# kevslinger/DTQN

Measured on AMD Instinct MI355X. Metric: env-steps/sec + TD-updates/sec, DiscreteCarFlag-v0 ctx=50 b=32, 1/2/4/8 GPU, higher is better.
Workload: dtype f32; 1 GPU; DiscreteCarFlag-v0 shapes (BASELINE config 1): ctx=50, d_model=64, 8 heads, 2 layers, obs 3 f32, 3 actions, batch 32 per GPU, history 50, device replay 2500 x 200 steps; global_batch=32, parallelism=dp1, sampler=device

## Files before the change

### dtqn_amd/csrc/dtqn_backward.hip

```cpp
#include "dtqn_device.hpp"
#include "dtqn_bwd_device.hpp"
#include "dtqn_gru.hpp"
#include "dtqn_wgrad_direct.hpp"
#include "dtqn_forward_body.hpp"

#ifndef DTQN_SPLIT_ATTN_MFMA
#define DTQN_SPLIT_ATTN_MFMA 1
#endif
#ifndef DTQN_BWD_DOX
#define DTQN_BWD_DOX 1
#endif
#ifndef DTQN_BWD_DOX_EARLY_FLAG
#define DTQN_BWD_DOX_EARLY_FLAG 1
#endif
#ifndef DTQN_BWD_FOLD_GUARD
#define DTQN_BWD_FOLD_GUARD 0
#endif
#if DTQN_BWD_FOLD_GUARD
#define DTQN_BWD_GUARD(w, q) Own::valid_fast(w, q)
#else
#define DTQN_BWD_GUARD(w, q) Own::valid(w, q)
#endif

namespace dtqn {

struct BwdArgs {
    DtqnNet net;
    const float* theta;
    const float* act;
    float* grd;
    float* small;
    const float* q3;
    float* stats_partial;
    const float* obs;
    const uint8_t* actions;
    const float* rewards;
    const uint8_t* dones;
    long long obs_ep_stride, act_ep_stride, rew_ep_stride;
    const int32_t* ep_idx;
    const int32_t* start;
    int batch, history;
    float gamma;
    long long* prof;
    float* xch;
    int32_t* xflags;
    uint32_t drop_thresh, drop_seed;
    float drop_scale;
    const int32_t* step_counter;
    FuseArgs fuse;
};

template <bool AHEAD> struct AheadArgs {};
template <> struct AheadArgs<true> { FwdArgs f; };

template <int D, int MT, int HD, int NW, bool GRU, int RS, bool DROP, bool FUSE = false, bool AHEAD = false, bool PAD = false>
__global__ __launch_bounds__(NW * 64) void dtqn_backward_kernel(BwdArgs a, AheadArgs<AHEAD> ahead) {
    static_assert(RS == 1 || RS == 2 || RS == 4, "one, two or four row slices");
    static_assert(!PAD || (RS == 4 && MT == 1 && !GRU && !DROP && !FUSE && D == 64), "width padding rides with the four-slice residual-gate chain");
    if constexpr (AHEAD) {
        static_assert(RS == 4 && MT == 1 && !GRU && !DROP && !FUSE && D <= 64, "the target pass ahead rides with the four-slice residual-gate chain");
        if ((int)blockIdx.x >= a.batch * RS) {
            forward_body_wl<D, 1, HD, NW, 4, false, PAD>(ahead.f);
            return;
        }
    }
    constexpr int NT = NW * 64;
    constexpr int LP = MT * 16;
    constexpr int LPF = LP * RS;
    constexpr int LDX = D + 4;
    constexpr int GW = D >= 64 ? 64 : D;
    constexpr int NG = D / GW;
    constexpr int NC = D >= 128 ? D / 2 : 2 * D;
    constexpr bool OST = D <= 64;
    constexpr int W5C = ((OST ? 6 : 5) * GW > NC ? (OST ? 6 : 5) * GW : NC);
    constexpr int LD5 = W5C + 4;
    constexpr int MGX = pick_mg(D / 16, MT, NW);
    using Own = Owned<D, MT, MGX, NW>;
    const DtqnNet& net = a.net;
    const Thr t = make_thr();
    const Thr& t_outer = t;
    if constexpr (FUSE) {
        if ((int)blockIdx.x >= a.batch * RS) {
            const DirectCtx ctx{a.act, a.grd, a.small, a.fuse.grad, a.batch, RS, a.fuse.n_small};
            fuse_role<NW>(net, a.fuse, ctx, (int)blockIdx.x - a.batch * RS, reinterpret_cast<float*>(dtqn_smem), t);
            return;
        }
    }
    int b, pos;
    slice_block_map((int)blockIdx.x, a.batch, RS, b, pos);
    const int slice = RS - 1 - pos;
    const int R0 = slice * LP;
    const int Lfull = net.ctx_len, A = net.num_actions, AP = net.ap, H = net.num_heads, adim = net.action_dim;
    const int L = Lfull - R0 < LP ? Lfull - R0 : LP;
    const bool ident = RS > 1 ? false : net.identity != 0;
    const int dreal = PAD ? net.d_real : D;
    constexpr bool gru = GRU;
    const float* __restrict__ theta = a.theta;
    const float* rec = a.act + (size_t)b * net.act_stride;
    float* grec = a.grd + (size_t)b * net.grd_stride;
    float* srec = a.small + ((size_t)b * RS + slice) * net.sp_stride;
    auto rf = [&](const float* base, int off, int w) -> const float* { return base + off + (size_t)R0 * w; };
    auto gf = [&](float* base, int off, int w) -> float* { return base + off + (size_t)R0 * w; };
    auto mf = [&](const float* base, int off, int ctiles) -> const float* { return base + off + (size_t)(R0 / 16) * ctiles * 8; };
    const DtqnRsrc grs = DTQN_XCH_RSRC(grec, (size_t)net.grd_stride * 4);
    constexpr bool WT = FUSE || (kOptBwdWT && !(GRU && !DROP && MT >= 2 && NW == 8));
    auto g_store4 = [&](float* p, float4 v) {
        if constexpr (WT) dtqn_xch_store4(grs, (int)(p - grec) * 4, v);
        else st4(p, v);
    };
    auto g_tile_store = [&](const float* s_, int ld_, float* g_, int rows, int cols, int gld = 0) {
        if constexpr (WT) {
            const int c4 = cols >> 2;
            if (gld == 0) gld = cols;
            const int base = (int)(g_ - grec);
            for (int idx = t_outer.tid; idx < rows * c4; idx += NT) {
                const int r = idx / c4, c = (idx - r * c4) * 4;
                dtqn_xch_store4(grs, (base + r * gld + c) * 4, ld4(s_ + r * ld_ + c));
            }
        } else {
            tile_store<NW>(s_, ld_, g_, rows, cols, t_outer, gld);
        }
    };
    auto s_store = [&](float* p, float v) {
        if constexpr (FUSE) DTQN_AGENT_STORE(p, v);
        else *p = v;
    };

    float* DX = reinterpret_cast<float*>(dtqn_smem);
    float* T2 = DX + LP * LDX;
    float* W5 = T2 + LP * LDX;
    float* dq_s = W5 + LPF * LD5;
    float* delta_s = dq_s + LP * AP;
    float* lse_s = delta_s + (GW / HD) * LPF;
    float* red = lse_s + (GW / HD) * LPF;
    constexpr int PARTS = NT / D >= 1 ? NT / D : 1;
    float* st_s = red + PARTS * 2 * D;
    float* DU = st_s + 4 * LP;

    const int ep = a.ep_idx[b], st0 = a.start[b] + R0;
    Drop dr = drop_off();
    if constexpr (DROP) dr = Drop{a.drop_thresh, a.drop_scale, a.drop_seed, (uint32_t)a.step_counter[1], (uint32_t)b};
    int ps = 0;
    DTQN_PROF(a.prof, ps++);
    static_assert(HD <= 16 || (HD == 32 && RS == 4 && MT == 1), "delta-in-epilogue: a head inside one 16-column tile, or two tiles wide on the four-slice chain");
    constexpr bool SPLITS = kOptSplitS && MT == 1 && 2 * (D / 16) == NW && 2 * (GW / 16) == NW;
    std::conditional_t<SPLITS, StageDyWSplit<D, NW, D / 16>, StageDyW<D, MT, pick_mg(D / 16, MT, NW), NW, D / 16>> g_h1;
    g_h1.prefetch(theta + net.off_head1_w, D, t);
    TileRegs<NW, LP, D> tr;
    TileRegs<NW, LP, D> trh;
    trh.load(rf(rec, net.ao_hh, D), D, t);
    if (!ident) tr.load(rf(rec, net.ao_layer0 + (net.num_layers - 1) * net.act_layer_stride + net.al_s2, D), D, t);

    static_assert(4 * LP <= NT, "one statistics value per thread");
    auto st_fetch = [&](int l) -> float {
        const float* lr = rec + net.ao_layer0 + (size_t)l * net.act_layer_stride;
        if (t.tid >= 4 * LP) return 0.f;
        return t.tid < 2 * LP ? rf(lr, net.al_st1, 2)[t.tid] : rf(lr, net.al_st2, 2)[t.tid - 2 * LP];
    };
    float st_next = st_fetch(net.num_layers - 1);

    {
        const float* q0 = a.q3 + (((size_t)0 * a.batch + b) * LPF + R0) * AP;
        const float* q1 = a.q3 + (((size_t)1 * a.batch + b) * LPF + R0) * AP;
        const float* q2 = a.q3 + (((size_t)2 * a.batch + b) * LPF + R0) * AP;
        const float inv_count = 1.0f / ((float)a.batch * (float)a.history);
        DTQN_PROF(a.prof, 24);
        for (int idx = t.tid; idx < LP * AP; idx += NT) dq_s[idx] = 0.f;
        __syncthreads();
        DTQN_PROF(a.prof, 25);
        if (t.wave == 0)
            td_loss_wave(q0, q1, q2, AP, A, Lfull - R0, LP, a.history, a.gamma, inv_count,
                         a.actions + (size_t)ep * a.act_ep_stride + st0, a.rewards + (size_t)ep * a.rew_ep_stride + st0,
                         a.dones + (size_t)ep * a.rew_ep_stride + st0, dq_s, a.stats_partial + ((size_t)b * RS + slice) * 8, t.lane);
        DTQN_PROF(a.prof, 26);
        __syncthreads();
        DTQN_PROF(a.prof, 27);
        if constexpr (WT) {
            for (int idx = t.tid; idx < LP * AP / 4; idx += NT) g_store4(gf(grec, net.go_dq, AP) + 4 * idx, ld4(dq_s + 4 * idx));
        } else {
            for (int idx = t.tid; idx < LP * AP; idx += NT) gf(grec, net.go_dq, AP)[idx] = dq_s[idx];
        }
    }

    DTQN_PROF(a.prof, ps++);
    {
        const float* __restrict__ W2 = theta + net.off_head2_w;
        constexpr int C4 = D / 4;
#pragma unroll
        for (int k4 = 0; k4 < TileRegs<NW, LP, D>::N; ++k4) {
            const int idx4 = t.tid + k4 * NT;
            if (idx4 < LP * C4) {
                const int r = idx4 / C4, c0 = (idx4 - r * C4) * 4;
                const float hv[4] = {trh.v[k4].x, trh.v[k4].y, trh.v[k4].z, trh.v[k4].w};
                float g4[4];
#pragma unroll
                for (int e = 0; e < 4; ++e) {
                    float g = 0.f;
                    if (hv[e] > 0.f)
                        for (int c = 0; c < A; ++c) g = fmaf(dq_s[r * AP + c], W2[c * D + c0 + e], g);
                    g4[e] = g;
                }
                st4(T2 + r * LDX + c0, make_float4(g4[0], g4[1], g4[2], g4[3]));
            }
        }
    }
    __syncthreads();
    g_h1.retire();
    g_tile_store(T2, LDX, gf(grec, net.go_dhh, D), LP, D);
    if constexpr (SPLITS) g_h1.run(T2, LDX, t, red, [&](int r, int c, float v) { DX[r * LDX + c] = v; });
    else g_h1.run(T2, LDX, t, [&](int r, int c, float v) { DX[r * LDX + c] = v; });
    __syncthreads();
    DTQN_PROF(a.prof, ps++);

    for (int l = net.num_layers - 1; l >= 0; --l) {
        Thr t = t_outer;
#define DTQN_RELAUNDER() do { if constexpr (D >= 128 && MT >= 4) { DTQN_ASM_KEEP(t.tid); DTQN_ASM_KEEP(t.lane); DTQN_ASM_KEEP(t.wave); DTQN_ASM_KEEP(t.i); DTQN_ASM_KEEP(t.kq); } \
        else if constexpr (D == 64 && MT >= 2 && NW <= 8 && (RS == 1 || (GRU && RS == 2))) { int tid_ = (int)threadIdx.x; DTQN_ASM_KEEP(tid_); t.tid = tid_; t.lane = tid_ & 63; t.wave = tid_ >> 6; t.i = t.lane & 15; t.kq = t.lane >> 4; } } while (0)
        DTQN_RELAUNDER();
        const float* __restrict__ th = layer_theta(net, theta, l);
        const float* lrec = rec + net.ao_layer0 + (size_t)l * net.act_layer_stride;
        float* lgrd = grec + net.go_layer0 + (size_t)l * net.grd_layer_stride;
        float* lsm = srec + net.so_ln + l * 4 * D;
        const float* __restrict__ W1 = th + net.lo_f1_w;
        const float* __restrict__ W2 = th + net.lo_f2_w;
        StageDyW<D, MT, pick_mg(NC / 16, MT, NW), NW, NC / 16> g_dh;
        g_dh.prefetch(W2, 4 * D, t);
        if (t.tid < 4 * LP) st_s[t.tid] = st_next;
        if (l > 0) st_next = st_fetch(l - 1);

        if (!ident) {
            if (l == net.num_layers - 1) DTQN_PROF(a.prof, 28);
            tr.to_lds(T2, LDX, t);
            if (l == net.num_layers - 1) DTQN_PROF(a.prof, 29);
            __syncthreads();
            if (l == net.num_layers - 1) DTQN_PROF(a.prof, 30);
            layernorm_backward<D, NW, FUSE, PAD>(DX, T2, DX, false, LDX, LP, st_s + 2 * LP, th + net.lo_ln2_w, lsm + 2 * D, red, t, false, dreal);
            if (l == net.num_layers - 1) DTQN_PROF(a.prof, 31);
            __syncthreads();
        }
        DTQN_PROF(a.prof, ps++);
        tr.load(rf(lrec, net.al_s1, D), D, t);
        if (gru) {
            gru_gate_backward<D, MT, NW>(DX, T2, LDX, W5, LD5, theta + net.off_gate_mlp, net, lrec + net.al_gate2, lgrd + net.gl_gate2, t, LPF, R0);
            __syncthreads();
        }
        {
            const float* m2 = mf(lrec, net.al_m2, D / 16);
            for (int idx = t.tid; idx < LP * D; idx += NT) {
                const int r = idx / D, c = idx - r * D;
                const float dy = gru ? T2[r * LDX + c] : DX[r * LDX + c];
                T2[r * LDX + c] = mask_bit(m2, D / 16, r, c) ? drop_apply(dr, DROP_FFN, l, (uint32_t)((R0 + r) * D + c), dy) : 0.f;
            }
        }
        __syncthreads();
        DTQN_RELAUNDER();
        {
            f32x4 xacc[Own::PER_WAVE][MGX];
#pragma unroll
            for (int q = 0; q < Own::PER_WAVE; ++q)
#pragma unroll
                for (int m = 0; m < MGX; ++m) xacc[q][m] = zero4();
            float w1f[2][NC / 4];
            constexpr bool SPLITK = kOptSplitK && Own::ITEMS * 2 == NW && Own::PER_WAVE == 1 && MGX == 1 && NC % 32 == 0;
            constexpr bool HALFW = kOptHalfW && !SPLITK && NC % 32 == 0;
            const int sk_it = t.wave % Own::ITEMS, sk_kh = t.wave / Own::ITEMS;
            const unsigned long long* mh = reinterpret_cast<const unsigned long long*>(mf(lrec, net.al_mh, 4 * D / 16));
            constexpr int MGH = pick_mg(NC / 16, MT, NW);
#pragma clang loop unroll_count(D >= 128 ? 1 : 4)
            for (int c0 = 0; c0 < 4 * D; c0 += NC) {
                g_dh.retire();
                if (c0 == 0) g_tile_store(T2, LDX, gf(lgrd, net.gl_df, D), LP, D);
                unsigned long long mw[MGH][4];
                g_dh.run(T2, LDX, t,
                         [&](int kt, int mg) {
#pragma unroll
                             for (int m = 0; m < MGH; ++m)
#pragma unroll
                                 for (int r = 0; r < 4; ++r)
                                     mw[m][r] = mh[((mg * MGH + m) * (4 * D / 16) + (c0 >> 4) + kt) * 4 + r];
                         },
                         [&](int r, int c, float v) {
                             const unsigned long long w = mw[(r >> 4) % MGH][r & 3];
                             W5[r * LD5 + c] = ((w >> t.lane) & 1ull) ? v : 0.f;
                         });
                if constexpr (SPLITK) {
                    float (&wh)[NC / 8] = *reinterpret_cast<float (*)[NC / 8]>(&w1f[0][0]);
                    frag_dyw_fetch<NC / 2>(wh, W1 + (size_t)(c0 + sk_kh * (NC / 2)) * D + sk_it * 16 + t.i, D, t);
                } else if constexpr (HALFW) {
                    float (&wh)[NC / 8] = *reinterpret_cast<float (*)[NC / 8]>(&w1f[0][0]);
                    if (DTQN_BWD_GUARD(t.wave, 0)) frag_dyw_fetch<NC / 2>(wh, W1 + (size_t)c0 * D + Own::nt(t.wave, 0) * 16 + t.i, D, t);
                } else if (DTQN_BWD_GUARD(t.wave, 0))
                    frag_dyw_fetch<NC>(w1f[0], W1 + (size_t)c0 * D + Own::nt(t.wave, 0) * 16 + t.i, D, t);
                if constexpr (FUSE) {
                    if (c0 == 0 && l + 1 < net.num_layers) DTQN_WAIT_VMEM();
                }
                __syncthreads();
                if constexpr (FUSE) {
                    if (c0 == 0 && l + 1 < net.num_layers) fuse_arrive(a.fuse.counters, net.num_layers - 2 - l, t);
                }
                if (SPLITK || DTQN_BWD_GUARD(t.wave, 0)) {
#pragma unroll
                    for (int q = 0; q < (SPLITK || HALFW ? NC / 8 : NC / 4); ++q) DTQN_ASM_KEEP(w1f[0][q]);
                }
                g_tile_store(W5, LD5, gf(lgrd, net.gl_dhp, 4 * D) + c0, LP, NC, 4 * D);
                if constexpr (SPLITK) {
                    const float (&wh)[NC / 8] = *reinterpret_cast<const float (*)[NC / 8]>(&w1f[0][0]);
                    frag_dyw_mma<NC / 2, 1>(W5 + sk_kh * (NC / 2), LD5, wh, t, xacc[0]);
                } else if constexpr (HALFW) {
                    float (&wa)[NC / 8] = *reinterpret_cast<float (*)[NC / 8]>(&w1f[0][0]);
                    float (&wb)[NC / 8] = *reinterpret_cast<float (*)[NC / 8]>(&w1f[1][0]);
#pragma unroll
                    for (int q = 0; q < Own::PER_WAVE; ++q) {
                        const float* wcol = W1 + (size_t)c0 * D + Own::nt(t.wave, q) * 16 + t.i;
                        const float* rows = W5 + Own::mg(t.wave, q) * MGX * 16 * LD5;
                        if (DTQN_BWD_GUARD(t.wave, q)) {
                            frag_dyw_fetch<NC / 2>(wb, wcol + (size_t)(NC / 2) * D, D, t);
                            frag_dyw_mma<NC / 2, MGX>(rows, LD5, wa, t, xacc[q]);
                        }
                        if (q + 1 < Own::PER_WAVE && DTQN_BWD_GUARD(t.wave, q + 1))
                            frag_dyw_fetch<NC / 2>(wa, W1 + (size_t)c0 * D + Own::nt(t.wave, q + 1) * 16 + t.i, D, t);
                        if (DTQN_BWD_GUARD(t.wave, q)) frag_dyw_mma<NC / 2, MGX>(rows + NC / 2, LD5, wb, t, xacc[q]);
                    }
                } else {
#pragma unroll
                    for (int q = 0; q < Own::PER_WAVE; ++q) {
                        if (q + 1 < Own::PER_WAVE && DTQN_BWD_GUARD(t.wave, q + 1))
                            frag_dyw_fetch<NC>(w1f[(q + 1) & 1], W1 + (size_t)c0 * D + Own::nt(t.wave, q + 1) * 16 + t.i, D, t);
                        if (DTQN_BWD_GUARD(t.wave, q))
                            frag_dyw_mma<NC, MGX>(W5 + Own::mg(t.wave, q) * MGX * 16 * LD5, LD5, w1f[q & 1], t, xacc[q]);
                    }
                }
                if (c0 + NC < 4 * D) g_dh.prefetch(W2 + c0 + NC, 4 * D, t);
                __syncthreads();
            }
            if constexpr (SPLITK) {
                if (t.wave >= Own::ITEMS) {
#pragma unroll
                    for (int r4 = 0; r4 < 4; ++r4) W5[((t.wave - Own::ITEMS) * 4 + r4) * 64 + t.lane] = xacc[0][0][r4];
                }
                __syncthreads();
                if (t.wave < Own::ITEMS) {
#pragma unroll
                    for (int r4 = 0; r4 < 4; ++r4) xacc[0][0][r4] += W5[(t.wave * 4 + r4) * 64 + t.lane];
                }
            }
            float* dst = ident ? DU : DX;
#pragma unroll
            for (int q = 0; q < Own::PER_WAVE; ++q) {
                if (DTQN_BWD_GUARD(t.wave, q)) {
                    const int c = Own::nt(t.wave, q) * 16 + t.i;
#pragma unroll
                    for (int m = 0; m < MGX; ++m)
#pragma unroll
                        for (int r4 = 0; r4 < 4; ++r4) {
                            const int r = (Own::mg(t.wave, q) * MGX + m) * 16 + t.kq * 4 + r4;
                            if (ident) dst[r * LDX + c] = xacc[q][m][r4];
                            else dst[r * LDX + c] += xacc[q][m][r4];
                        }
                }
            }
        }
        tr.to_lds(T2, LDX, t);
        constexpr bool DOX = RS > 1 && DTQN_BWD_DOX && DTQN_SPLIT_ATTN_MFMA;
        TileRegs<NW, LP, GW> tq, to, tk[RS], tv[RS], tqu[DOX ? RS : 1];
        constexpr int NLSE = (GW / HD) * LPF, LSE_N = (NLSE + NT - 1) / NT;
        float lse_r[LSE_N];
        auto load_group = [&](int g) {
            if constexpr (kOptLse) {
#pragma unroll
                for (int k = 0; k < LSE_N; ++k) {
                    const int idx = t.tid + k * NT;
                    lse_r[k] = lrec[net.al_lse + g * NLSE + (idx < NLSE ? idx : 0)];
                }
            }
            const float* qkv0 = lrec + net.al_qkv + g * GW;
            tq.load(qkv0 + (size_t)R0 * 3 * D, 3 * D, t);
            if constexpr (DOX) {
#pragma unroll
                for (int j = 1; j < RS; ++j)
                    if (j > slice) tqu[j].load(qkv0 + (size_t)j * LP * 3 * D, 3 * D, t);
            }
#pragma unroll
            for (int j = 0; j < RS; ++j)
                if (j <= slice) {
                    tk[j].load(qkv0 + (size_t)j * LP * 3 * D + D, 3 * D, t);
                    tv[j].load(qkv0 + (size_t)j * LP * 3 * D + 2 * D, 3 * D, t);
                }
            if (OST) to.load(rf(lrec, net.al_o, D) + g * GW, D, t);
        };
        load_group(0);
        const float* __restrict__ Wo = th + net.lo_out_w;
        const float* __restrict__ Win = th + net.lo_in_w;
        std::conditional_t<SPLITS, StageDyWSplit<D, NW, GW / 16>, StageDyW<D, MT, pick_mg(GW / 16, MT, NW), NW, GW / 16>> g_do;
// ... 169 lines not shown
                        const DtqnRsrc rs = DTQN_XCH_RSRC(xg + (size_t)pair_id(slice, 0) * LP * 2 * GW, R0 * 2 * GW * 4);
                        constexpr int C4 = 2 * GW / 4;
                        for (int idx = t.tid; idx < R0 * C4; idx += NT) {
                            const int r = idx / C4, c = (idx - r * C4) * 4;
                            dtqn_xch_store4(rs, idx * 16, ld4(W5 + r * LD5 + GW + c));
                        }
                        DTQN_WAIT_VMEM();
                        __syncthreads();
                        if (t.tid < slice) DTQN_AGENT_STORE(fg + pair_id(slice, t.tid), (int32_t)1);
                    }
                    for (int sndr = slice + 1; sndr < RS; ++sndr)
                        xch_recv<NW, true>(W5r + GW, LD5, xg + (size_t)pair_id(sndr, slice) * LP * 2 * GW, LP, 2 * GW,
                                           fg + pair_id(sndr, slice), t);
                }
                }
                DTQN_PROF(a.prof, ps++);
                if constexpr (SPLITW) {
#pragma unroll
                    for (int q = 0; q < WPC / 4; ++q) DTQN_ASM_KEEP(wpc[0][q]);
                } else if (DTQN_BWD_GUARD(t.wave, 0)) {
#pragma unroll
                    for (int q = 0; q < GW / 4; ++q) DTQN_ASM_KEEP(winf[0][q]);
                }
                if (g == 0 && DOX) g_tile_store(T2, LDX, gf(lgrd, net.gl_da, D), LP, D);
                for (int idx = t.tid; idx < LP * 3 * (GW / 4); idx += NT) {
                    const int r = idx / (3 * (GW / 4)), rem = idx - r * (3 * (GW / 4));
                    const int which = rem / (GW / 4), c = (rem - which * (GW / 4)) * 4;
                    const float* sp = W5r + r * LD5 + (which == 0 ? 4 * GW : which * GW) + c;
                    g_store4(gf(lgrd, net.gl_dqkv, 3 * D) + (size_t)r * 3 * D + which * D + g * GW + c, ld4(sp));
                }
                if constexpr (SPLITW) {
#pragma unroll
                    for (int j = 0; j < 3; ++j) {
                        if (j + 1 < 3) piece_fetch(wpc[(j + 1) & 1], g, j + 1);
                        const int u = sw_kh * 3 + j, part = u >> 1, off = (u & 1) * WPC;
                        frag_dyw_mma<WPC, 1>(W5r + (part == 0 ? 4 * GW : part * GW) + off, LD5, wpc[j & 1], t, xacc[0]);
                    }
                } else
#pragma unroll
                for (int q = 0; q < Own::PER_WAVE; ++q) {
#pragma unroll
                    for (int part = 0; part < 3; ++part) {
                        const int step = q * 3 + part;
                        const int nq = part < 2 ? q : q + 1, np = part < 2 ? part + 1 : 0;
                        if (nq < Own::PER_WAVE && DTQN_BWD_GUARD(t.wave, nq))
                            frag_dyw_fetch<GW>(winf[(step + 1) & 1], Win + (size_t)(np * D + g * GW) * D + Own::nt(t.wave, nq) * 16 + t.i, D, t);
                        if (DTQN_BWD_GUARD(t.wave, q)) {
                            const float* rows = W5r + Own::mg(t.wave, q) * MGX * 16 * LD5 + (part == 0 ? 4 * GW : part * GW);
                            frag_dyw_mma<GW, MGX>(rows, LD5, winf[step & 1], t, xacc[q]);
                        }
                    }
                }
                if (g + 1 < NG) {
                    g_do.prefetch(Wo + (g + 1) * GW, D, t);
                    load_group(g + 1);
                }
                __syncthreads();
            }
            if (!ident) {
                if (l > 0) tr.load(rf(rec, net.ao_layer0 + (l - 1) * net.act_layer_stride + net.al_s2, D), D, t);
            } else {
                tr.load(l == 0 ? rf(rec, net.ao_x0, D) : rf(rec, net.ao_layer0 + (l - 1) * net.act_layer_stride + net.al_s2, D), D, t);
            }
            if constexpr (SPLITW) {
                if (t.wave >= Own::ITEMS) {
#pragma unroll
                    for (int r4 = 0; r4 < 4; ++r4) W5[((t.wave - Own::ITEMS) * 4 + r4) * 64 + t.lane] = xacc[0][0][r4];
                }
                __syncthreads();
                if (t.wave < Own::ITEMS) {
#pragma unroll
                    for (int r4 = 0; r4 < 4; ++r4) xacc[0][0][r4] += W5[(t.wave * 4 + r4) * 64 + t.lane];
                }
            }
            float* dst = ident ? DU : DX;
#pragma unroll
            for (int q = 0; q < Own::PER_WAVE; ++q) {
                if (DTQN_BWD_GUARD(t.wave, q)) {
                    const int c = Own::nt(t.wave, q) * 16 + t.i;
#pragma unroll
                    for (int m = 0; m < MGX; ++m)
#pragma unroll
                        for (int r4 = 0; r4 < 4; ++r4) {
                            const int r = (Own::mg(t.wave, q) * MGX + m) * 16 + t.kq * 4 + r4;
                            if (ident) dst[r * LDX + c] = xacc[q][m][r4];
                            else dst[r * LDX + c] += xacc[q][m][r4];
                        }
                }
            }
        }
        __syncthreads();
        DTQN_PROF(a.prof, ps++);
        if (ident) {
            tr.to_lds(T2, LDX, t);
            __syncthreads();
            layernorm_backward<D, NW, FUSE, PAD>(DU, T2, DX, true, LDX, LP, st_s, th + net.lo_ln1_w, lsm, red, t, false, dreal);
            __syncthreads();
        }
    }

    DTQN_PROF(a.prof, ps++);
    if (dr.thresh != 0u) {
        for (int idx = t.tid; idx < LP * D; idx += NT) {
            const int r = idx / D, c = idx - r * D;
            DX[r * LDX + c] = drop_apply(dr, DROP_EMB, 0, (uint32_t)((R0 + r) * D + c), DX[r * LDX + c]);
        }
        __syncthreads();
    }
    g_tile_store(DX, LDX, gf(grec, net.go_dx0, D), LP, D);
    const float* obs_rows = a.obs + (size_t)ep * a.obs_ep_stride + (size_t)st0 * net.obs_dim;
    const uint8_t* act_rows = a.actions + (size_t)ep * a.act_ep_stride + st0;
    if (net.discrete) {
        const int KE = net.ke, KEP = net.kep, e = net.embed_per_obs, V = net.vocab, O = net.obs_dim;
        const float* __restrict__ We = theta + net.off_obs_w;
        float* dein = W5;
        for (int idx = t.tid; idx < LP * KEP; idx += NT) {
            const int r = idx / KEP, k = idx - r * KEP;
            float g = 0.f;
            if (r < L && k < KE)
                for (int d = 0; d < D - adim; ++d) g = fmaf(DX[r * LDX + adim + d], We[(size_t)d * KE + k], g);
            dein[idx] = g;
        }
        __syncthreads();
        for (int idx = t.tid; idx < V * e; idx += NT) {
            const int v = idx / e, c = idx - v * e;
            float g = 0.f;
            for (int r = 0; r < L; ++r)
                for (int j = 0; j < O; ++j) {
                    int tok = (int)obs_rows[(size_t)r * O + j];
                    tok = tok < 0 ? 0 : (tok >= V ? V - 1 : tok);
                    if (tok == v) g += dein[r * KEP + j * e + c];
                }
            s_store(srec + net.so_tab + idx, g);
        }
    }
    if (adim > 0) {
        for (int idx = t.tid; idx < A * adim; idx += NT) {
            const int v = idx / adim, c = idx - v * adim;
            float g = 0.f;
            if (Lfull == 1) {
                if ((int)act_rows[0] == v) g = DX[c];
            } else {
                for (int r = R0 > 0 ? 0 : 1; r < L; ++r)
                    if ((int)act_rows[r - 1] == v) g += DX[r * LDX + c];
            }
            s_store(srec + net.so_act + idx, g);
        }
    }
    if constexpr (FUSE) {
        DTQN_WAIT_VMEM();
        __syncthreads();
        fuse_arrive(a.fuse.counters, net.num_layers, t);
    }
}

static size_t bwd_lds_bytes(const DtqnNet* net) {
    const int LP = net->lp, D = net->d_model, HD = net->head_dim;
    const int GW = D >= 64 ? 64 : D, NC = D >= 128 ? D : 2 * D;
    const int ntile = D <= 64 ? 6 : 5;
    const int W5C = ntile * GW > NC ? ntile * GW : NC;
    const int NT = waves_for(*net) * 64;
    const int PARTS = NT / D >= 1 ? NT / D : 1;
    size_t fl = 2 * (size_t)LP * (D + 4) + (size_t)LP * (W5C + 4) + (size_t)LP * net->ap + 2 * (size_t)(GW / HD) * LP +
                (size_t)PARTS * 2 * D + 4 * (size_t)LP;
    if (net->identity) fl += (size_t)LP * (D + 4);
    return fl * sizeof(float);
}

template <int D, int MT, int HD, int NW, bool GRU, int RS, bool DROP, bool FUSE = false>
static int launch_bwd3(const BwdArgs& a, hipStream_t stream) {
    const size_t lds = bwd_lds_bytes(&a.net);
    static size_t attr_lds[kMaxDevices] = {};
    raise_lds_limit(reinterpret_cast<const void*>(&dtqn_backward_kernel<D, MT, HD, NW, GRU, RS, DROP, FUSE>), lds, attr_lds);
    (void)hipGetLastError();
    const int grid = a.batch * RS + (FUSE ? a.fuse.n_role : 0);
    hipLaunchKernelGGL((dtqn_backward_kernel<D, MT, HD, NW, GRU, RS, DROP, FUSE>), dim3(grid), dim3(NW * 64), lds, stream, a, AheadArgs<false>{});
    return hipGetLastError() == hipSuccess ? DTQN_OK : DTQN_ERR_LAUNCH;
}
template <int HD, bool PAD = false>
static int launch_bwd_ahead(const BwdArgs& a, const FwdArgs& f, hipStream_t stream) {
    const size_t lb = bwd_lds_bytes(&a.net), lf = fwd_lds_bytes(&a.net, true);
    const size_t lds = lb > lf ? lb : lf;
    if (lds > 160 * 1024) return DTQN_ERR_CONFIG;
    static size_t attr_lds[kMaxDevices] = {};
    raise_lds_limit(reinterpret_cast<const void*>(&dtqn_backward_kernel<64, 1, HD, 8, false, 4, false, false, true, PAD>), lds, attr_lds);
    (void)hipGetLastError();
    AheadArgs<true> ah;
    ah.f = f;
    ah.f.block0 = a.batch * 4;
    hipLaunchKernelGGL((dtqn_backward_kernel<64, 1, HD, 8, false, 4, false, false, true, PAD>), dim3(a.batch * 4 + f.batch * 4), dim3(8 * 64), lds, stream, a, ah);
    return hipGetLastError() == hipSuccess ? DTQN_OK : DTQN_ERR_LAUNCH;
}
template <int HD, bool PAD>
static int launch_bwd_lite(const BwdArgs& a, hipStream_t stream) {
    const size_t lds = bwd_lds_bytes(&a.net);
    static size_t attr_lds[kMaxDevices] = {};
    raise_lds_limit(reinterpret_cast<const void*>(&dtqn_backward_kernel<64, 1, HD, 8, false, 4, false, false, false, PAD>), lds, attr_lds);
    (void)hipGetLastError();
    hipLaunchKernelGGL((dtqn_backward_kernel<64, 1, HD, 8, false, 4, false, false, false, PAD>), dim3(a.batch * 4), dim3(8 * 64), lds, stream, a, AheadArgs<false>{});
    return hipGetLastError() == hipSuccess ? DTQN_OK : DTQN_ERR_LAUNCH;
}
template <int D, int MT, int HD, int NW, bool GRU, int RS>
static int launch_bwd2(const BwdArgs& a, hipStream_t stream) {
    if constexpr (RS == 4 && !GRU && NW == kFuseWaves) {
        if (a.fuse.n_role > 0) {
            if (bwd_lds_bytes(&a.net) < (kFuseWaves + (size_t)(kDSmallFused / 64) * kFuseWaves * 64) * sizeof(float) ||
                bwd_lds_bytes(&a.net) < direct_lds_floats(kFuseWaves) * sizeof(float)) return DTQN_ERR_CONFIG;
            if (a.drop_thresh != 0u) return launch_bwd3<D, MT, HD, NW, GRU, RS, true, true>(a, stream);
            return launch_bwd3<D, MT, HD, NW, GRU, RS, false, true>(a, stream);
        }
    }
    if (a.fuse.n_role > 0) return DTQN_ERR_CONFIG;
    if (a.drop_thresh != 0u) return launch_bwd3<D, MT, HD, NW, GRU, RS, true>(a, stream);
    return launch_bwd3<D, MT, HD, NW, GRU, RS, false>(a, stream);
}
template <int D, int MT, int HD, int NW>
static int launch_bwd(const BwdArgs& a, hipStream_t stream) {
    if (a.net.gate == DTQN_GATE_GRU) {
        if constexpr (D <= 64) return launch_bwd2<D, MT, HD, NW, true, 1>(a, stream);
        else return DTQN_ERR_CONFIG;
    }
    return launch_bwd2<D, MT, HD, NW, false, 1>(a, stream);
}

}

using namespace dtqn;

extern "C" int dtqn_lds_bytes_backward(const DtqnNet* net) {
    if (!net) return 0;
    const size_t b = bwd_lds_bytes(net);
    return b <= 160 * 1024 ? (int)b : 0;
}

extern "C" int dtqn_td_wgrad_is_fused(const DtqnNet* net, const DtqnTd* td) {
    FuseArgs f;
    return fuse_plan(net, td, &f) ? 1 : 0;
}

static int td_backward(const DtqnNet* net, const DtqnReplay* rp, const DtqnTd* td, const DtqnTd* td_next, int draw_step_next, void* stream);

extern "C" int dtqn_td_backward(const DtqnNet* net, const DtqnReplay* rp, const DtqnTd* td, void* stream) {
    return td_backward(net, rp, td, nullptr, -1, stream);
}

extern "C" int dtqn_td_backward_ahead(const DtqnNet* net, const DtqnReplay* rp, const DtqnTd* td, const DtqnTd* td_next, int draw_step_next,
                                      void* stream) {
    if (!td_next || draw_step_next < 0) return DTQN_ERR_ARG;
    return td_backward(net, rp, td, td_next, draw_step_next, stream);
}

static int td_backward(const DtqnNet* net, const DtqnReplay* rp, const DtqnTd* td, const DtqnTd* td_next, int draw_step_next, void* stream) {
    if (!net || !rp || !td || td->batch < 1) return DTQN_ERR_ARG;
    if (td->history < 1 || td->history > net->ctx_len) return DTQN_ERR_ARG;
    if (net->tiled) return td_next ? DTQN_ERR_CONFIG : tiled_td_backward(net, rp, td, (hipStream_t)stream);
    if (bwd_lds_bytes(net) > 160 * 1024) return DTQN_ERR_CONFIG;
    BwdArgs a;
    a.net = *net;
    a.theta = td->theta_pol;
    a.act = td->act; a.grd = td->grd; a.small = td->small; a.q3 = td->q3; a.stats_partial = td->stats_partial;
    a.obs = rp->obs; a.actions = rp->actions; a.rewards = rp->rewards; a.dones = rp->dones;
    a.obs_ep_stride = (long long)(rp->max_steps + 1) * rp->obs_dim;
    a.act_ep_stride = rp->max_steps + 1;
    a.rew_ep_stride = rp->max_steps;
    a.ep_idx = td->ep_idx; a.start = td->start;
    a.batch = td->batch; a.history = td->history; a.gamma = td->gamma;
    a.prof = dtqn_debug_profile_buffer() ? static_cast<long long*>(dtqn_debug_profile_buffer()) + 64 : nullptr;
    a.xch = td->xch; a.xflags = td->xflags;
    a.drop_thresh = net->dropout > 0.f ? (uint32_t)((double)net->dropout * 4294967296.0) : 0u;
    a.drop_scale = net->dropout > 0.f ? 1.0f / (1.0f - net->dropout) : 1.0f;
    a.drop_seed = td->dropout_seed; a.step_counter = td->step_counter;
    fuse_plan(net, td, &a.fuse);
    const int D = net->d_model, MT = net->lp / 16, HD = net->head_dim, NW = waves_for(*net);
    hipStream_t s = (hipStream_t)stream;
    if (dtqn_ws_lite(net->tiled, D, HD, net->d_real)) {
        if (td->row_split != 4 || net->lp != 64 || net->identity || net->gate != DTQN_GATE_RES || !a.xch || !a.xflags || a.drop_thresh != 0u ||
            a.fuse.n_role > 0 || NW != 8) return DTQN_ERR_CONFIG;
        const bool pad = net->d_real > 0;
        if (td_next != nullptr) {
            if (!dtqn_td_fwd_slices4_ok(net) || !td_next->sample_in_kernel || td_next->batch != td->batch || !td_next->xch || !td_next->xflags ||
                !td_next->q3) return DTQN_ERR_CONFIG;
            FwdArgs f;
            td_forward_args(net, rp, td_next, 2, draw_step_next, &f);
            f.nseq = td_next->batch;
            f.prof = nullptr;
            if (HD == 8 && pad) return launch_bwd_ahead<8, true>(a, f, s);
            if (HD == 16 && pad) return launch_bwd_ahead<16, true>(a, f, s);
            if (HD == 32) return pad ? launch_bwd_ahead<32, true>(a, f, s) : launch_bwd_ahead<32, false>(a, f, s);
            return DTQN_ERR_CONFIG;
        }
        if (HD == 8 && pad) return launch_bwd_lite<8, true>(a, s);
        if (HD == 16 && pad) return launch_bwd_lite<16, true>(a, s);
        if (HD == 32) return pad ? launch_bwd_lite<32, true>(a, s) : launch_bwd_lite<32, false>(a, s);
        return DTQN_ERR_CONFIG;
    }
    if (td->row_split == 2 || td->row_split == 4) {
        if (net->lp != 64 || net->identity || !a.xch || !a.xflags) return DTQN_ERR_CONFIG;
        if (net->gate == DTQN_GATE_GRU) {
            if (td->row_split == 4) {
                if (D == 64 && HD == 8) return launch_bwd2<64, 1, 8, 8, true, 4>(a, s);
                if (D == 64 && HD == 16) return launch_bwd2<64, 1, 16, 8, true, 4>(a, s);
                return DTQN_ERR_CONFIG;
            }
            if (D == 64 && HD == 8) return launch_bwd2<64, 2, 8, 8, true, 2>(a, s);
            if (D == 64 && HD == 16) return launch_bwd2<64, 2, 16, 8, true, 2>(a, s);
            return DTQN_ERR_CONFIG;
// ... 31 lines not shown
```

### dtqn_amd/csrc/dtqn_bwd_device.hpp

```cpp
#pragma once
#include "dtqn_device.hpp"

namespace dtqn {

template <int D, int NW, bool WT = false, bool PAD = false>
__device__ __forceinline__ void layernorm_backward(const float* dy, const float* xin, float* dst, bool accumulate,
                                                   int ld, int LP, const float* __restrict__ st,
                                                   const float* __restrict__ gamma, float* __restrict__ dgb,
                                                   float* red, const Thr& t, bool dgb_accumulate = false, int d_real = D) {
    constexpr int NT = NW * 64;
    constexpr int PARTS = NT / D >= 1 ? NT / D : 1;
    {
        const int d = t.tid % D, part = t.tid / D;
        if (part < PARTS) {
            float sg = 0.f, sb = 0.f;
            for (int r = part; r < LP; r += PARTS) {
                const float mean = st[r * 2], rstd = st[r * 2 + 1];
                const float g = dy[r * ld + d];
                sg = fmaf(g, (xin[r * ld + d] - mean) * rstd, sg);
                sb += g;
            }
            red[(part * 2 + 0) * D + d] = sg;
            red[(part * 2 + 1) * D + d] = sb;
        }
// ... 230 lines not shown
    bool one_round = nblocks <= NW && (64 % HG) == 0;
    int nlive = ((q_hi > row0 ? q_hi - row0 : 0) * HG + 63) / 64;
    for (int it0 = t.tid; it0 < (one_round ? NW * 64 : LP * HG); it0 += NW * 64) {
        int item = it0;
        if (one_round) {
            const int blk = balanced_block<NW>(t.wave, nblocks, nlive, false);
            if (blk < 0) continue;
            item = blk * 64 + t.lane;
            if (item >= LP * HG) continue;
        }
        const int rl = item / HG, hl = item - rl * HG;
        const int row = row0 + rl;
        float* dqp = dq_base + (size_t)row * dq_ld + hl * HD;
        float dq[HD];
#pragma unroll
        for (int c = 0; c < HD; ++c) dq[c] = 0.f;
        if (row < n) {
            const float* qp = W5 + row * ld + hl * HD;
            const float* dop = W5 + row * ld + 3 * GW + hl * HD;
            float q[HD], dO[HD];
#pragma unroll
            for (int c = 0; c < HD; c += 4) {
                const float4 x = ld4(qp + c), g = ld4(dop + c);
                q[c] = x.x * scale; q[c + 1] = x.y * scale; q[c + 2] = x.z * scale; q[c + 3] = x.w * scale;
                dO[c] = g.x; dO[c + 1] = g.y; dO[c + 2] = g.z; dO[c + 3] = g.w;
            }
            const float delta = delta_s[hl * sl_ld + row], lse = lse_s[hl * sl_ld + row];
            const float* kbase = W5 + GW + hl * HD;
            for (int s = 0; s <= row; ++s) {
                const float* kp = kbase + s * ld;
                const float* vp = kp + GW;
                float sc = 0.f, dp = 0.f;
                float kk[HD];
#pragma unroll
                for (int c = 0; c < HD; c += 4) {
                    const float4 k = ld4(kp + c), v = ld4(vp + c);
                    kk[c] = k.x; kk[c + 1] = k.y; kk[c + 2] = k.z; kk[c + 3] = k.w;
                    sc = fmaf(q[c], k.x, sc); sc = fmaf(q[c + 1], k.y, sc); sc = fmaf(q[c + 2], k.z, sc); sc = fmaf(q[c + 3], k.w, sc);
                    dp = fmaf(dO[c], v.x, dp); dp = fmaf(dO[c + 1], v.y, dp); dp = fmaf(dO[c + 2], v.z, dp); dp = fmaf(dO[c + 3], v.w, dp);
                }
                if (dr.thresh != 0u) dp = drop_keep(dr, DROP_ATTN, layer, drop_attn_idx(head0 + hl, row, s)) ? dp * dr.scale : 0.f;
                const float ds = __expf(sc - lse) * (dp - delta);
#pragma unroll
                for (int c = 0; c < HD; ++c) dq[c] = fmaf(ds, kk[c], dq[c]);
            }
        }
#pragma unroll
        for (int c = 0; c < HD; c += 4)
            st4(dqp + c, make_float4(dq[c] * scale, dq[c + 1] * scale, dq[c + 2] * scale, dq[c + 3] * scale));
    }
    __syncthreads();
    const int KR = row0 + LP;
    nblocks = (KR * HG + 63) / 64;
    one_round = nblocks <= NW && (64 % HG) == 0;
    nlive = ((q_hi < KR ? q_hi : KR) * HG + 63) / 64;
    for (int it0 = t.tid; it0 < (one_round ? NW * 64 : KR * HG); it0 += NW * 64) {
        int item = it0;
        if (one_round) {
            const int blk = balanced_block<NW>(t.wave, nblocks, nlive, true);
            if (blk < 0) continue;
            item = blk * 64 + t.lane;
            if (item >= KR * HG) continue;
        }
        const int srow = item / HG, hl = item - srow * HG;
        float* kp = W5 + srow * ld + GW + hl * HD;
        float* vp = kp + GW;
        float dk[HD], dv[HD];
#pragma unroll
        for (int c = 0; c < HD; ++c) dk[c] = dv[c] = 0.f;
        if (srow < q_hi) {
            float k[HD], v[HD];
#pragma unroll
            for (int c = 0; c < HD; c += 4) {
                const float4 x = ld4(kp + c), y = ld4(vp + c);
                k[c] = x.x; k[c + 1] = x.y; k[c + 2] = x.z; k[c + 3] = x.w;
                v[c] = y.x; v[c + 1] = y.y; v[c + 2] = y.z; v[c + 3] = y.w;
            }
            const int q_lo = srow > row0 ? srow : row0;
            for (int row = q_hi - 1; row >= q_lo; --row) {
                const float* qp = W5 + row * ld + hl * HD;
                const float* dop = qp + 3 * GW;
                float sc = 0.f, dp = 0.f;
                float qq[HD], dd[HD];
#pragma unroll
                for (int c = 0; c < HD; c += 4) {
                    const float4 x = ld4(qp + c), g = ld4(dop + c);
                    qq[c] = x.x * scale; qq[c + 1] = x.y * scale; qq[c + 2] = x.z * scale; qq[c + 3] = x.w * scale;
                    dd[c] = g.x; dd[c + 1] = g.y; dd[c + 2] = g.z; dd[c + 3] = g.w;
                }
#pragma unroll
                for (int c = 0; c < HD; ++c) { sc = fmaf(qq[c], k[c], sc); dp = fmaf(dd[c], v[c], dp); }
                float p = __expf(sc - lse_s[hl * sl_ld + row]);
                float pv = p;
                if (dr.thresh != 0u) {
                    const bool keep = drop_keep(dr, DROP_ATTN, layer, drop_attn_idx(head0 + hl, row, srow));
                    dp = keep ? dp * dr.scale : 0.f;
                    pv = keep ? p * dr.scale : 0.f;
                }
                const float ds = p * (dp - delta_s[hl * sl_ld + row]);
#pragma unroll
                for (int c = 0; c < HD; ++c) { dk[c] = fmaf(ds, qq[c], dk[c]); dv[c] = fmaf(pv, dd[c], dv[c]); }
            }
        }
#pragma unroll
        for (int c = 0; c < HD; c += 4) {
            st4(kp + c, make_float4(dk[c], dk[c + 1], dk[c + 2], dk[c + 3]));
            st4(vp + c, make_float4(dv[c], dv[c + 1], dv[c + 2], dv[c + 3]));
        }
    }
}

template <int HD, int NW, bool MFMA = (HD >= kAttnMfmaMinHeadDim)>
__device__ __forceinline__ void attention_backward_group(float* W5, int ld, int GW, int LP, int n,
                                                         const float* delta_s, const float* lse_s, const Thr& t,
                                                         float* dq_base = nullptr, int dq_ld = 0, int row0 = 0, int sl_ld = 0,
                                                         const Drop& dr = Drop{0u, 1.0f, 0u, 0u, 0u}, int layer = 0, int head0 = 0,
                                                         float hd_eff = (float)HD) {
    if constexpr (MFMA)
        attention_backward_group_mfma<HD, NW>(W5, ld, GW, LP, n, delta_s, lse_s, t, dq_base, dq_ld, row0, sl_ld, dr, layer, head0, false, 0,
                                              AttnNoBetween(), hd_eff);
    else attention_backward_group_valu<HD, NW>(W5, ld, GW, LP, n, delta_s, lse_s, t, dq_base, dq_ld, row0, sl_ld, dr, layer, head0, hd_eff);
}

__device__ __forceinline__ void td_loss_wave(const float* q0, const float* q1, const float* q2, int AP, int A, int L, int LPB,
                                             int history, float gamma, float inv_count, const uint8_t* act, const float* rew,
                                             const uint8_t* don, float* dq, float* sp, int lane) {
    float sq = 0.f, mnq = INFINITY, mxq = -INFINITY, sy = 0.f, mny = INFINITY, mxy = -INFINITY, se = 0.f;
    for (int r = lane; r < LPB; r += 64) {
        if (r < L && r >= L - history) {
            const int at = (int)act[r];
            const float rw = rew[r];
            const float dn = don[r] ? 1.f : 0.f;
            float q = 0.f, best = q1[r * AP], qt = q2[r * AP];
            for (int c = 0; c < A; ++c) {
                const float v0 = q0[r * AP + c], v1 = q1[r * AP + c], v2 = q2[r * AP + c];
                if (c == at) q = v0;
                if (c > 0 && v1 > best) { best = v1; qt = v2; }
            }
            const float y = rw + (1.f - dn) * (qt * gamma);
            const float diff = q - y;
            dq[r * AP + at] = 2.f * diff * inv_count;
            sq += q; mnq = fminf(mnq, q); mxq = fmaxf(mxq, q);
            sy += y; mny = fminf(mny, y); mxy = fmaxf(mxy, y);
            se = fmaf(diff, diff, se);
        }
    }
    sq = wave_sum(sq); sy = wave_sum(sy); se = wave_sum(se);
    mnq = wave_min(mnq); mxq = wave_max(mxq); mny = wave_min(mny); mxy = wave_max(mxy);
    if (lane == 0) {
        sp[0] = se; sp[1] = sq; sp[2] = mxq; sp[3] = mnq; sp[4] = sy; sp[5] = mxy; sp[6] = mny; sp[7] = 0.f;
    }
}

}
```

Measured before the change: 12170 TD-updates/s.

## Split TD loss into early load issue and late finish; stage head.2 weights in LDS

The TD-loss global loads (Q values, actions, rewards, dones) are issued at kernel entry so they overlap the weight prefetches, and the loss is computed later from registers. This drops the separate dq zero-fill pass and one barrier, since each lane now writes its whole dq row. The head.2 weight matrix is staged in LDS, and the head gradient is computed as a float4 FMA with the ReLU mask applied afterwards instead of a per-element branch. Profiling timestamps are collected into a local clock array and written out at kernel end. The trade-off is extra register pressure from holding the loss operands across the prefetch phase.

```diff
diff --git a/dtqn_amd/csrc/dtqn_backward.hip b/dtqn_amd/csrc/dtqn_backward.hip
--- a/dtqn_amd/csrc/dtqn_backward.hip
+++ b/dtqn_amd/csrc/dtqn_backward.hip
@@ -140,8 +140,26 @@
     const int ep = a.ep_idx[b], st0 = a.start[b] + R0;
     Drop dr = drop_off();
     if constexpr (DROP) dr = Drop{a.drop_thresh, a.drop_scale, a.drop_seed, (uint32_t)a.step_counter[1], (uint32_t)b};
-    int ps = 0;
-    DTQN_PROF(a.prof, ps++);
+    enum { PK_ENTRY, PK_PREFETCH, PK_LOSS_LOADS, PK_LOSS_WAVE, PK_LOSS_BARRIER, PK_LOSS, PK_HEAD2, PK_HEAD, PK_DH_PREFETCH,
+           PK_STATS, PK_S2_BEFORE, PK_S2_LDS, PK_S2_BARRIER, PK_LN2_BODY, PK_LN2, PK_N };
+    long long pclk[PK_N] = {};
+    int ps = 4;
+    DTQN_PROF_CLOCK(pclk[PK_ENTRY]);
+    static_assert(LP <= 64, "one loss row per lane of one wave");
+    const float* q0 = a.q3 + (((size_t)0 * a.batch + b) * LPF + R0) * AP;
+    const float* q1 = a.q3 + (((size_t)1 * a.batch + b) * LPF + R0) * AP;
+    const float* q2 = a.q3 + (((size_t)2 * a.batch + b) * LPF + R0) * AP;
+    TdLossRow lrow = {};
+    if (t.wave == 0)
+        td_loss_issue(lrow, q0, q1, q2, AP, Lfull - R0, LP, a.history, -R0,
+                      a.actions + (size_t)ep * a.act_ep_stride + st0, a.rewards + (size_t)ep * a.rew_ep_stride + st0,
+                      a.dones + (size_t)ep * a.rew_ep_stride + st0, t.lane);
+    DTQN_SCHED_FENCE();
+    DTQN_PROF_CLOCK(pclk[PK_LOSS_LOADS]);
+    const float* __restrict__ W2h = theta + net.off_head2_w;
+    const int h2n4 = A * (D / 4);
+    static_assert(LPF * LD5 >= DTQN_MAX_ACTIONS * D, "head.2 fits the wide temp");
+    const float4 h2 = ld4(W2h + 4 * (t.tid < h2n4 ? t.tid : 0));
     static_assert(HD <= 16 || (HD == 32 && RS == 4 && MT == 1), "delta-in-epilogue: a head inside one 16-column tile, or two tiles wide on the four-slice chain");
     constexpr bool SPLITS = kOptSplitS && MT == 1 && 2 * (D / 16) == NW && 2 * (GW / 16) == NW;
     std::conditional_t<SPLITS, StageDyWSplit<D, NW, D / 16>, StageDyW<D, MT, pick_mg(D / 16, MT, NW), NW, D / 16>> g_h1;
@@ -160,21 +178,15 @@
     float st_next = st_fetch(net.num_layers - 1);
 
     {
-        const float* q0 = a.q3 + (((size_t)0 * a.batch + b) * LPF + R0) * AP;
-        const float* q1 = a.q3 + (((size_t)1 * a.batch + b) * LPF + R0) * AP;
-        const float* q2 = a.q3 + (((size_t)2 * a.batch + b) * LPF + R0) * AP;
         const float inv_count = 1.0f / ((float)a.batch * (float)a.history);
-        DTQN_PROF(a.prof, 24);
-        for (int idx = t.tid; idx < LP * AP; idx += NT) dq_s[idx] = 0.f;
+        DTQN_PROF_CLOCK(pclk[PK_PREFETCH]);
+        if (t.wave == 0)
+            td_loss_finish(lrow, q0, q1, q2, AP, A, LP, a.gamma, inv_count, dq_s, a.stats_partial + ((size_t)b * RS + slice) * 8, t.lane);
+        DTQN_PROF_CLOCK(pclk[PK_LOSS_WAVE]);
+        if (t.tid < h2n4) st4(W5 + 4 * t.tid, h2);
+        for (int idx = t.tid + NT; idx < h2n4; idx += NT) st4(W5 + 4 * idx, ld4(W2h + 4 * idx));
         __syncthreads();
-        DTQN_PROF(a.prof, 25);
-        if (t.wave == 0)
-            td_loss_wave(q0, q1, q2, AP, A, Lfull - R0, LP, a.history, a.gamma, inv_count,
-                         a.actions + (size_t)ep * a.act_ep_stride + st0, a.rewards + (size_t)ep * a.rew_ep_stride + st0,
-                         a.dones + (size_t)ep * a.rew_ep_stride + st0, dq_s, a.stats_partial + ((size_t)b * RS + slice) * 8, t.lane);
-        DTQN_PROF(a.prof, 26);
-        __syncthreads();
-        DTQN_PROF(a.prof, 27);
+        DTQN_PROF_CLOCK(pclk[PK_LOSS_BARRIER]);
         if constexpr (WT) {
             for (int idx = t.tid; idx < LP * AP / 4; idx += NT) g_store4(gf(grec, net.go_dq, AP) + 4 * idx, ld4(dq_s + 4 * idx));
         } else {
@@ -182,35 +194,33 @@
         }
     }
 
-    DTQN_PROF(a.prof, ps++);
+    DTQN_PROF_CLOCK(pclk[PK_LOSS]);
     {
-        const float* __restrict__ W2 = theta + net.off_head2_w;
         constexpr int C4 = D / 4;
 #pragma unroll
         for (int k4 = 0; k4 < TileRegs<NW, LP, D>::N; ++k4) {
             const int idx4 = t.tid + k4 * NT;
             if (idx4 < LP * C4) {
                 const int r = idx4 / C4, c0 = (idx4 - r * C4) * 4;
-                const float hv[4] = {trh.v[k4].x, trh.v[k4].y, trh.v[k4].z, trh.v[k4].w};
-                float g4[4];
-#pragma unroll
-                for (int e = 0; e < 4; ++e) {
-                    float g = 0.f;
-                    if (hv[e] > 0.f)
-                        for (int c = 0; c < A; ++c) g = fmaf(dq_s[r * AP + c], W2[c * D + c0 + e], g);
-                    g4[e] = g;
-                }
-                st4(T2 + r * LDX + c0, make_float4(g4[0], g4[1], g4[2], g4[3]));
-            }
-        }
-    }
+                float4 g = make_float4(0.f, 0.f, 0.f, 0.f);
+                for (int c = 0; c < A; ++c) {
+                    const float d = dq_s[r * AP + c];
+                    const float4 w = ld4(W5 + c * D + c0);
+                    g.x = fmaf(d, w.x, g.x); g.y = fmaf(d, w.y, g.y); g.z = fmaf(d, w.z, g.z); g.w = fmaf(d, w.w, g.w);
+                }
+                const float4 hv = trh.v[k4];
+                st4(T2 + r * LDX + c0, make_float4(hv.x > 0.f ? g.x : 0.f, hv.y > 0.f ? g.y : 0.f, hv.z > 0.f ? g.z : 0.f, hv.w > 0.f ? g.w : 0.f));
+            }
+        }
+    }
+    DTQN_PROF_CLOCK(pclk[PK_HEAD2]);
     __syncthreads();
     g_h1.retire();
     g_tile_store(T2, LDX, gf(grec, net.go_dhh, D), LP, D);
     if constexpr (SPLITS) g_h1.run(T2, LDX, t, red, [&](int r, int c, float v) { DX[r * LDX + c] = v; });
     else g_h1.run(T2, LDX, t, [&](int r, int c, float v) { DX[r * LDX + c] = v; });
     __syncthreads();
-    DTQN_PROF(a.prof, ps++);
+    DTQN_PROF_CLOCK(pclk[PK_HEAD]);
 
     for (int l = net.num_layers - 1; l >= 0; --l) {
         Thr t = t_outer;
@@ -225,20 +235,23 @@
         const float* __restrict__ W2 = th + net.lo_f2_w;
         StageDyW<D, MT, pick_mg(NC / 16, MT, NW), NW, NC / 16> g_dh;
         g_dh.prefetch(W2, 4 * D, t);
+        if (l == net.num_layers - 1) DTQN_PROF_CLOCK(pclk[PK_DH_PREFETCH]);
         if (t.tid < 4 * LP) st_s[t.tid] = st_next;
         if (l > 0) st_next = st_fetch(l - 1);
+        if (l == net.num_layers - 1) DTQN_PROF_CLOCK(pclk[PK_STATS]);
 
         if (!ident) {
-            if (l == net.num_layers - 1) DTQN_PROF(a.prof, 28);
+            if (l == net.num_layers - 1) DTQN_PROF_CLOCK(pclk[PK_S2_BEFORE]);
             tr.to_lds(T2, LDX, t);
-            if (l == net.num_layers - 1) DTQN_PROF(a.prof, 29);
+            if (l == net.num_layers - 1) DTQN_PROF_CLOCK(pclk[PK_S2_LDS]);
             __syncthreads();
-            if (l == net.num_layers - 1) DTQN_PROF(a.prof, 30);
+            if (l == net.num_layers - 1) DTQN_PROF_CLOCK(pclk[PK_S2_BARRIER]);
             layernorm_backward<D, NW, FUSE, PAD>(DX, T2, DX, false, LDX, LP, st_s + 2 * LP, th + net.lo_ln2_w, lsm + 2 * D, red, t, false, dreal);
-            if (l == net.num_layers - 1) DTQN_PROF(a.prof, 31);
+            if (l == net.num_layers - 1) DTQN_PROF_CLOCK(pclk[PK_LN2_BODY]);
             __syncthreads();
         }
-        DTQN_PROF(a.prof, ps++);
+        if (l == net.num_layers - 1) DTQN_PROF_CLOCK(pclk[PK_LN2]);
+        else DTQN_PROF(a.prof, ps++);
         tr.load(rf(lrec, net.al_s1, D), D, t);
         if (gru) {
             gru_gate_backward<D, MT, NW>(DX, T2, LDX, W5, LD5, theta + net.off_gate_mlp, net, lrec + net.al_gate2, lgrd + net.gl_gate2, t, LPF, R0);
@@ -714,6 +727,11 @@
         __syncthreads();
         fuse_arrive(a.fuse.counters, net.num_layers, t);
     }
+    {
+        constexpr int slot_of[PK_N] = {0, 24, 20, 26, 27, 1, 21, 2, 22, 23, 28, 29, 30, 31, 3};
+#pragma unroll
+        for (int k = 0; k < PK_N; ++k) DTQN_PROF_PUT(a.prof, slot_of[k], pclk[k]);
+    }
 }
 
 static size_t bwd_lds_bytes(const DtqnNet* net) {
diff --git a/dtqn_amd/csrc/dtqn_bwd_device.hpp b/dtqn_amd/csrc/dtqn_bwd_device.hpp
--- a/dtqn_amd/csrc/dtqn_bwd_device.hpp
+++ b/dtqn_amd/csrc/dtqn_bwd_device.hpp
@@ -406,4 +406,74 @@
     }
 }
 
-}
+constexpr int kLossQ4 = 2;
+struct TdLossRow {
+    bool live;
+    int at;
+    float rw;
+    int dn;
+    float4 v0[kLossQ4], v1[kLossQ4], v2[kLossQ4];
+};
+__device__ __forceinline__ void td_loss_issue(TdLossRow& w, const float* q0, const float* q1, const float* q2, int AP, int L, int LPB,
+                                              int history, int stand_in, const uint8_t* act, const float* rew, const uint8_t* don, int lane) {
+    w.live = lane < LPB && lane < L && lane >= L - history;
+    const int r = w.live ? lane : stand_in;
+    w.at = (int)act[r];
+    w.rw = rew[r];
+    w.dn = (int)don[r];
+#pragma unroll
+    for (int k = 0; k < kLossQ4; ++k) {
+        const int c = 4 * k < AP ? 4 * k : 0;
+        w.v0[k] = ld4(q0 + r * AP + c);
+        w.v1[k] = ld4(q1 + r * AP + c);
+        w.v2[k] = ld4(q2 + r * AP + c);
+    }
+}
+__device__ __forceinline__ void td_loss_finish(const TdLossRow& w, const float* q0, const float* q1, const float* q2, int AP, int A, int LPB,
+                                               float gamma, float inv_count, float* dq, float* sp, int lane) {
+    float sq = 0.f, mnq = INFINITY, mxq = -INFINITY, sy = 0.f, mny = INFINITY, mxy = -INFINITY, se = 0.f;
+    int at = -1;
+    float g = 0.f;
+    if (w.live) {
+        at = w.at;
+        const float rw = w.rw;
+        const float dn = w.dn ? 1.f : 0.f;
+        float e0[4 * kLossQ4], e1[4 * kLossQ4], e2[4 * kLossQ4];
+#pragma unroll
+        for (int k = 0; k < kLossQ4; ++k) {
+            e0[4 * k] = w.v0[k].x; e0[4 * k + 1] = w.v0[k].y; e0[4 * k + 2] = w.v0[k].z; e0[4 * k + 3] = w.v0[k].w;
+            e1[4 * k] = w.v1[k].x; e1[4 * k + 1] = w.v1[k].y; e1[4 * k + 2] = w.v1[k].z; e1[4 * k + 3] = w.v1[k].w;
+            e2[4 * k] = w.v2[k].x; e2[4 * k + 1] = w.v2[k].y; e2[4 * k + 2] = w.v2[k].z; e2[4 * k + 3] = w.v2[k].w;
+        }
+        float q = 0.f, best = e1[0], qt = e2[0];
+#pragma unroll
+        for (int c = 0; c < 4 * kLossQ4; ++c) {
+            if (c < A) {
+                if (c == at) q = e0[c];
+                if (c > 0 && e1[c] > best) { best = e1[c]; qt = e2[c]; }
+            }
+        }
+        for (int c = 4 * kLossQ4; c < A; ++c) {
+            const float v0 = q0[lane * AP + c], v1 = q1[lane * AP + c], v2 = q2[lane * AP + c];
+            if (c == at) q = v0;
+            if (v1 > best) { best = v1; qt = v2; }
+        }
+        const float y = rw + (1.f - dn) * (qt * gamma);
+        const float diff = q - y;
+        g = 2.f * diff * inv_count;
+        sq += q; mnq = fminf(mnq, q); mxq = fmaxf(mxq, q);
+        sy += y; mny = fminf(mny, y); mxy = fmaxf(mxy, y);
+        se = fmaf(diff, diff, se);
+    }
+    if (lane < LPB) {
+        for (int c = 0; c < AP; c += 4)
+            st4(dq + lane * AP + c, make_float4(c == at ? g : 0.f, c + 1 == at ? g : 0.f, c + 2 == at ? g : 0.f, c + 3 == at ? g : 0.f));
+    }
+    sq = wave_sum(sq); sy = wave_sum(sy); se = wave_sum(se);
+    mnq = wave_min(mnq); mxq = wave_max(mxq); mny = wave_min(mny); mxy = wave_max(mxy);
+    if (lane == 0) {
+        sp[0] = se; sp[1] = sq; sp[2] = mxq; sp[3] = mnq; sp[4] = sy; sp[5] = mxy; sp[6] = mny; sp[7] = 0.f;
+    }
+}
+
+}
```

Measured after the change: 12310 TD-updates/s, median of 6. 1.1% higher.
